# 10183308/popsift

Hardware: AMD Instinct MI355X
Metric: Mpix/s SIFT extract on 1920x1080 (keypoints+descriptors) (higher is better)
Workload: dtype f32; 1 GPU; 1920x1080 u8 grayscale, default popsift::Config (2x upscale, 9 octaves, 3 levels, PopSift mode, loop descriptor, RootSift); distinct_images_per_gpu=16, contexts_per_gpu=3, images_per_launch=16

## Files before the change

### popsift_amd/csrc/keypoint.hip

```cpp
#include <hip/hip_runtime.h>

#include "kernels.h"
#include "sift_types.h"

namespace popsift_hip {
namespace {

constexpr float F_PI = 3.14159265358979323846f;
constexpr float F_PI2 = 2.0f * 3.14159265358979323846f;
constexpr float            ORI_WINFACTOR = 1.5f;
constexpr float            DESC_MAGNIFY = 3.0f;

typedef unsigned long long fix64;
__device__ __forceinline__ fix64 to_fix(float w) { return (fix64)(unsigned int)(w * 1048576.0f); }
__device__ __forceinline__ float from_fix(fix64 v) { return (float)((double)v * (1.0 / 1048576.0)); }


__device__ __forceinline__ void wave_lds_sync()
{
    __builtin_amdgcn_fence(__ATOMIC_SEQ_CST, "wavefront");
    __builtin_amdgcn_wave_barrier();
}

__device__ __forceinline__ int wave_incl_scan(int v)
// ... 162 lines not shown
    return copysignf(2.0f - b, y);
}

__device__ __forceinline__ float atan2_bins(float y, float x)
{
    const float ax = fabsf(x), ay = fabsf(y);
    const float mx = fmaxf(fmaxf(ax, ay), 1e-30f), mn = fminf(ax, ay);
    const float r = mn * __builtin_amdgcn_rcpf(mx);
    const float s = r * r;
    float       p = fmaf(-0.01492126751691103f, s, 0.06703268736600876f);
    p = fmaf(p, s, -0.14823880791664124f);
    p = fmaf(p, s, 0.24642325937747955f);
    p = fmaf(p, s, -0.42350852489471436f);
    p = fmaf(p, s, 1.2732105255126953f);
    return octants(p * r, x, y, ax, ay);
}

__device__ __forceinline__ float atan2_bins9(float y, float x)
{
    const float ax = fabsf(x), ay = fabsf(y);
    const float mx = fmaxf(fmaxf(ax, ay), 1e-30f), mn = fminf(ax, ay);
    const float r = mn * __builtin_amdgcn_rcpf(mx);
    const float s = r * r;
    float       p = fmaf(0.026540832594037056f, s, -0.1084246039390564f);
    p = fmaf(p, s, 0.22938621044158936f);
    p = fmaf(p, s, -0.4205572307109833f);
    p = fmaf(p, s, 1.2730693817138672f);
    return octants(p * r, x, y, ax, ay);
}

typedef float v2f __attribute__((ext_vector_type(2)));
typedef __attribute__((address_space(3))) fix64 lds_fix64;
typedef __attribute__((address_space(3))) unsigned int lds_u32;

#ifndef KP_NW
#define KP_NW 1
#endif
constexpr int ORI_COPIES = 4;

__global__ __launch_bounds__(64 * KP_NW) void k_orientation(const PyrDesc* __restrict__ pdp, BatchDesc bd, SiftConsts sc,
                                                     int filtered, int hist_cap)
{
    const float* __restrict__   arena = bd.s[blockIdx.y].arena;
    Counters* __restrict__      ct = bd.s[blockIdx.y].ct;
    const InitExt* __restrict__ iext = filtered ? bd.s[blockIdx.y].iext2 : bd.s[blockIdx.y].iext;
    float* __restrict__         ohist = bd.s[blockIdx.y].ohist;
    const int n_oct = pdp->n_oct, L = pdp->L;
    constexpr int    NB = PS_ORI_NBINS + 2;
    __shared__ fix64 s_hist[KP_NW][ORI_COPIES][NB];
    const int        wave = threadIdx.x >> 6, lane = threadIdx.x & 63;
    fix64*           hall = &s_hist[wave][0][0];
    fix64*           hist = s_hist[wave][lane & (ORI_COPIES - 1)];

    __shared__ int ps[PS_MAX_OCT + 1];
    if (threadIdx.x == 0) ext_prefix(ct, sc, n_oct, ps);
    __syncthreads();
    const int total = min(ps[n_oct], hist_cap);

    for (XcdSlice sl = xcd_slice<KP_NW>(); sl.more(total); sl.s += sl.step) {
        const int g = sl.index();
        if (g >= total) continue;
        int o = 0;
        while (o + 1 < n_oct && g >= ps[o + 1]) o++;
        o = uniform(o);
        const InitExt  ie = iext[(size_t)o * sc.max_extrema + (g - uniform(ps[o]))];
        const OctDesc* od = &pdp->o[o];
// ... 170 lines not shown
        } else {
            angle_out[k] = 0.0f;
        }
    }
    return angles;
}

__device__ __forceinline__ DescRec make_desc_rec(const PyrDesc* __restrict__ pdp, const Ext& e, float angle, float cos_t, float sin_t)
{
    DescRec        r;
    const OctDesc* od = &pdp->o[e.octave];
    const int      lvl = min(max(e.lpos, 0), pdp->L - 1);
    const long long off = od->data_off + lvl * od->plane_stride;
    const float    x = e.xpos, y = e.ypos;
    const float    SBP = fabsf(DESC_MAGNIFY * e.sigma);
    const float    cell_px = (2.83f * SBP + 1.0f) * (2.83f * SBP + 1.0f);
    const int      fbits = min(max(31 - (int)ceilf(log2f(361.0f * cell_px)), 2), 14);
    const float    csbp = cos_t * SBP, ssbp = sin_t * SBP;
    const float    bsz = fabsf(csbp) + fabsf(ssbp);
    const float    ext_r = 2.5f * bsz;
    const int      xmin = max(1, (int)floorf(x - ext_r));
    const int      ymin = max(1, (int)floorf(y - ext_r));
    const int      xmax = min(od->w - 2, (int)floorf(x + ext_r) + 1);
    const int      ymax = min(od->h - 2, (int)floorf(y + ext_r) + 1);
    r.x = x;
    r.y = y;
    r.crsbp = cos_t / SBP;
    r.srsbp = sin_t / SBP;
    r.ang_bins = angle * (4.0f / F_PI);
    r.inv_c = (fabsf(r.crsbp) > 1e-20f) ? __builtin_amdgcn_rcpf(r.crsbp) : 0.0f;
    r.inv_s = (fabsf(r.srsbp) > 1e-20f) ? __builtin_amdgcn_rcpf(r.srsbp) : 0.0f;
    r.xymin = ((unsigned int)xmin & 0xffffu) | ((unsigned int)ymin << 16);
    r.xymax = ((unsigned int)xmax & 0xffffu) | ((unsigned int)ymax << 16);
    r.off_lo = (unsigned int)((unsigned long long)off & 0xffffffffull);
    r.off_hi = (unsigned int)((unsigned long long)off >> 32);
    r.misc = (unsigned int)od->pitch | ((unsigned int)fbits << 16) | ((SBP != 0.0f) ? (1u << 24) : 0u);
    return r;
}


constexpr int SCAN_ITEMS = 1;
constexpr int SCAN_CHUNK = 256 * SCAN_ITEMS;
constexpr int SCAN_LT = 256;
constexpr int SCAN_LCHUNK = SCAN_LT / 4;
constexpr int SCAN_SUB = SCAN_CHUNK / SCAN_LCHUNK;

__device__ __forceinline__ int clamped_total(const Counters* ct, const SiftConsts& sc, int n_oct)
{
    int acc = 0;
    for (int o = 0; o < n_oct; o++) acc += min(ct->ext_ct[o], sc.max_extrema);
    return acc;
}

__global__ __launch_bounds__(SCAN_LT) void k_scan_local(const PyrDesc* __restrict__ pdp, SiftConsts sc, BatchDesc bd,
                                                     int filtered, int hist_cap)
{
    const Counters* __restrict__ ct = bd.s[blockIdx.y].ct;
    const InitExt* __restrict__  iext = filtered ? bd.s[blockIdx.y].iext2 : bd.s[blockIdx.y].iext;
    const float* __restrict__    ohist = bd.s[blockIdx.y].ohist;
    Ext* __restrict__            ext = bd.s[blockIdx.y].ext;
    int* __restrict__            partial = bd.s[blockIdx.y].partial;
    static_assert(SCAN_CHUNK % SCAN_LCHUNK == 0 && SCAN_LT % 64 == 0, "four lanes per extremum, whole waves");
    __shared__ int s_wsum[SCAN_LT / 64];
    __shared__ int s_ps[PS_MAX_OCT + 1];
    const int      n_oct = pdp->n_oct;
    if (threadIdx.x == 0) ext_prefix(ct, sc, n_oct, s_ps);
    __syncthreads();
    const int total = s_ps[n_oct];
    const int tid = threadIdx.x, lane = tid & 63, wave = tid >> 6;
// ... 105 lines not shown
                    map[idx + q] = g;
                    float sn, cs;
                    sincos_cr(e.orientation[q], sn, cs);
                    rot[idx + q] = make_float2(cs, sn);
                    if (drec) drec[idx + q] = make_desc_rec(pdp, e, e.orientation[q], cs, sn);
                }
            }
            feats[g] = f;
            for (int o = 0; o < n_oct; o++)
                if (g == s_ps[o] && s_ps[o + 1] > s_ps[o]) ct->ori_ps[o] = idx;
        }
    }
    if (tid == 0 && chunk == nb - 1) {
        int last = chunk_offset;
        for (int k = 0; k < SCAN_SUB && (chunk * SCAN_SUB + k) * SCAN_LCHUNK < total; k++) last += partial[chunk * SCAN_SUB + k];
        ct->ori_total = last;
        ct->ext_total = total;
        for (int o = 0; o < PS_MAX_OCT; o++) {
            ct->ext_ct[o] = (o < n_oct) ? min(ct->ext_ct[o], sc.max_extrema) : 0;
            ct->ext_ps[o] = s_ps[o];
        }
    }
    __syncthreads();
    }
}


#ifndef DESC_NCOPY
#define DESC_NCOPY 4
#endif
constexpr int DESC_COPIES = DESC_NCOPY;
constexpr int DESC_RS = 36;
constexpr int DESC_CS = 3 * DESC_RS + 32;
constexpr int DESC_MAXROWS = 128;

__global__ __launch_bounds__(64 * KP_NW, 8) void k_descriptor(BatchDesc bd, SiftConsts sc, int desc_cap)
{
    const float* __restrict__   arena = bd.s[blockIdx.y].arena;
    const Counters* __restrict__ ct = bd.s[blockIdx.y].ct;
    const DescRec* __restrict__ drec = bd.s[blockIdx.y].drec;
    float* __restrict__         desc = bd.s[blockIdx.y].desc;
    constexpr int ROW_WORDS = (DESC_MAXROWS + 1 + 3) & ~3;
    static_assert(ROW_WORDS * 4 >= 352, "cell (-1, -1) of copy 0 stays inside the wave's LDS");
    __shared__ __attribute__((aligned(16))) unsigned int s_lds[KP_NW][ROW_WORDS + 2 * DESC_COPIES * DESC_CS];
    const int     lane = threadIdx.x & 63, wave = threadIdx.x >> 6;
    const int     cpy = lane & (DESC_COPIES - 1);
    unsigned int* rinfo = s_lds[wave];
    fix64*        hall = (fix64*)(s_lds[wave] + ROW_WORDS);
    const unsigned int rbase32 = (unsigned int)(size_t)(lds_u32*)rinfo;
    const float        hbasef = (float)(unsigned int)(size_t)(lds_fix64*)(hall + cpy * DESC_CS);
    const float        cpy8f = (float)(cpy << 3);
    const int     total = min(ct->ori_total, desc_cap);
    const int     maxrows = min(max(sc.desc_rows, 4), DESC_MAXROWS);

    for (XcdSlice sl = xcd_slice<KP_NW>(); sl.more(total); sl.s += sl.step) {
        const int d = sl.index();
        if (d >= total) continue;
        typedef unsigned int u4 __attribute__((ext_vector_type(4)));
        const u4*          rp = reinterpret_cast<const u4*>(drec + d);
        const u4           q0 = rp[0], q1 = rp[1], q2 = rp[2];
        const float        x = uniformf(__uint_as_float(q0.x)), y = uniformf(__uint_as_float(q0.y));
        const float        crsbp = uniformf(__uint_as_float(q0.z)), srsbp = uniformf(__uint_as_float(q0.w));
        const float        ang_bins = uniformf(__uint_as_float(q1.x));
        const float        inv_c = uniformf(__uint_as_float(q1.y)), inv_s = uniformf(__uint_as_float(q2.w));
        const int          pmin = uniform((int)q1.z), pmax = uniform((int)q1.w);
        const unsigned int misc = (unsigned int)uniform((int)q2.z);
        const int          pitch = (int)(misc & 0xffffu), fbits = (int)((misc >> 16) & 0xffu);
        const float*       layer = arena + uniform64((long long)(((unsigned long long)q2.y << 32) | q2.x));

        {
            u4 zero;
            asm volatile("v_mov_b32 %0, 0\n\tv_mov_b32 %1, 0\n\tv_mov_b32 %2, 0\n\tv_mov_b32 %3, 0"
                         : "=v"(zero.x), "=v"(zero.y), "=v"(zero.z), "=v"(zero.w));
            constexpr int CLEAR16 = DESC_COPIES * DESC_CS / 2;
            static_assert(DESC_COPIES * DESC_CS % 2 == 0, "whole 16-byte pieces");
            u4*           h16 = reinterpret_cast<u4*>(hall);
#pragma unroll
            for (int k = 0; k < (CLEAR16 + 63) / 64; k++)
                if (lane + 64 * k < CLEAR16) h16[lane + 64 * k] = zero;
        }

        if (misc & (1u << 24)) {
            const int   xmin = (int)(short)(pmin & 0xffff), ymin0 = pmin >> 16;
            const int   xmax = (int)(short)(pmax & 0xffff), ymax = pmax >> 16;
            const int   wx = xmax - xmin + 1;
            const int   hy_all = ymax - ymin0 + 1;
            const float ffbits = (float)fbits;

            for (int rb = 0; rb < hy_all && wx > 0; rb += maxrows) {
            const int   ymin = ymin0 + rb;
            const int   hy = min(hy_all - rb, maxrows);

            int T = 0, grow = 0;
            {
                int         carry = 0;
                for (int r0 = 0; r0 < hy; r0 += 64) {
                    const int r = r0 + lane;
                    int       len = 0, jlo = xmin;
                    if (r < hy) {
                        const float dy = (float)(ymin + r) - y;
                        const float a = srsbp * dy, b = crsbp * dy;
                        float       lo = -1e30f, hi = 1e30f;
                        bool        ok = true;
                        if (inv_c != 0.0f) {
                            const float t0 = (-2.5f - a) * inv_c, t1 = (2.5f - a) * inv_c;
                            lo = fminf(t0, t1);
                            hi = fmaxf(t0, t1);
                        } else {
                            ok = fabsf(a) < 2.5f;
                        }
                        if (inv_s != 0.0f) {
                            const float t0 = (b - 2.5f) * inv_s, t1 = (b + 2.5f) * inv_s;
                            lo = fmaxf(lo, fminf(t0, t1));
                            hi = fminf(hi, fmaxf(t0, t1));
                        } else {
                            ok = ok && (fabsf(b) < 2.5f);
                        }
                        jlo = max(xmin, (int)floorf(x + lo - 1e-3f) + 1);
                        const int jhi = min(xmax, (int)ceilf(x + hi + 1e-3f) - 1);
                        len = ok ? max(jhi - jlo + 1, 0) : 0;
                        if (len == 0) jlo = xmin;
                    }
                    const int incl = wave_incl_scan(len);
                    const int start = carry + incl - len;
                    if (r < hy) rinfo[r] = (unsigned int)start | ((unsigned int)(start - (jlo - xmin)) << 16);
                    const unsigned long long live = __ballot(len > 0);
                    if (carry == 0 && live != 0ull) grow = r0 + __ffsll((long long)live) - 1;
                    carry += __builtin_amdgcn_readlane(incl, 63);
                }
                T = carry;
                if (lane == 0) {
                    rinfo[hy] = (unsigned int)T | 0x7fff0000u;
                    rinfo[hy + 1] = 0xffffu;
                }
            }
            wave_lds_sync();

#ifdef DESC_PROBE_NOLOOP
            const int   steps = 0;
#else
            const int   steps = (T + 63) >> 6;
#endif
            unsigned int rp = rbase32 + 4u * (unsigned int)grow;
            float        fr = (float)(rb + grow);
            unsigned int cur = 0;
            unsigned int nxt = 0x7fff0000u | 0xffffu;
            if (T > 0) {
                cur = rinfo[grow];
                nxt = rinfo[grow + 1];
            }

            const float  ox = (float)xmin - x, oy = (float)ymin0 - y;
            const float  u0 = fmaf(crsbp, ox, srsbp * oy), v0 = fmaf(crsbp, oy, -srsbp * ox);
            const float* corner = layer + (size_t)(ymin0 * pitch + xmin);
            const float  pitch4f = (float)(4 * pitch);

            auto coord = [&](int i, unsigned int& off, float& u, float& v) {
                while (i >= (int)(nxt & 0xffffu)) {
                    fr += 1.0f;
                    rp += 4u;
                    cur = nxt;
                    nxt = *(lds_u32*)(size_t)(rp + 4u);
                }
                const float fc = (float)(i - ((int)cur >> 16));
                u = fmaf(crsbp, fc, fmaf(srsbp, fr, u0));
                v = fmaf(crsbp, fr, fmaf(-srsbp, fc, v0));
                asm("v_cvt_u32_f32 %0, %1" : "=v"(off) : "v"(fmaf(fr, pitch4f, fc * 4.0f)));
            };
            unsigned int probe_acc = 0u;
            auto bin = [&](float u, float v, float gx, float gy) {
                if (fabsf(u) < 2.5f && fabsf(v) < 2.5f) {
                    const float  mod = __builtin_amdgcn_sqrtf(fmaf(gx, gx, gy * gy));
                    const float  wm = __builtin_amdgcn_exp2f(fmaf(-0.18033688011112042f, fmaf(u, u, v * v), ffbits)) * mod;
                    const float tth = atan2_bins9(gy, gx) - ang_bins;
                    const float ffo = floorf(tth);
                    const float do0 = tth - ffo;

                    const float tu = u + 1.5f, tv = v + 1.5f;
                    const float fcx = floorf(tu), fcy = floorf(tv);
                    const float fx = tu - fcx, fy = tv - fcy;
                    const float wx0 = 1.0f - fx, wy0 = (1.0f - fy) * wm, wy1 = fy * wm;
                    const float w0 = 1.0f - do0;
                    const unsigned int s0 = (unsigned int)(int)fmaf(fcx, 32.0f, fmaf(ffo, 8.0f, cpy8f)) & 56u;
                    const unsigned int cb = (unsigned int)(int)fmaf(fcy, (float)(DESC_RS * 8), fmaf(fcx, 64.0f, hbasef));
                    const unsigned int e0 = cb + s0;
                    const unsigned int e1 = (s0 ^ 32u) + cb;
                    const bool x0 = tu >= 0.0f, x1 = tu < 3.0f, y0 = tv >= 0.0f, y1 = tv < 3.0f;
#ifdef DESC_PROBE_NOATOMIC
#define PS_CELL_ADD(ADDR, LO, HI) probe_acc ^= (LO) ^ (HI) ^ (ADDR);
#else
#define PS_CELL_ADD(ADDR, LO, HI)                                                                             \
    __hip_atomic_fetch_add((lds_fix64*)(size_t)(ADDR), ((fix64)(HI) << 32) | (fix64)(LO), __ATOMIC_RELAXED,    \
                           __HIP_MEMORY_SCOPE_WORKGROUP);
#endif
#define PS_CELL(ADDR, WGT)                                                                                     \
    {                                                                                                          \
        const float        wgt = (WGT);                                                                        \
        const unsigned int lo = __float_as_uint(fmaf(w0, wgt, 8388608.0f)) & 0x7fffffu;                        \
        const unsigned int hi = __float_as_uint(fmaf(do0, wgt, 8388608.0f)) & 0x7fffffu;                       \
        PS_CELL_ADD(ADDR, lo, hi)                                                                              \
    }
                    if (y0) {
                        if (x0) PS_CELL(e0, wy0 * wx0)
                        if (x1) PS_CELL(e1 + 64u, wy0 * fx)
                    }
                    if (y1) {
                        if (x0) PS_CELL(e0 + DESC_RS * 8u, wy1 * wx0)
                        if (x1) PS_CELL(e1 + DESC_RS * 8u + 64u, wy1 * fx)
                    }
#undef PS_CELL
#undef PS_CELL_ADD
                }
            };
            unsigned int off_a = 0, off_b = 0;
            float u_a = 3.0f, v_a = 3.0f, a0 = 0.0f, a1 = 0.0f, a2 = 0.0f, a3 = 0.0f;
            float u_b = 3.0f, v_b = 3.0f, b0 = 0.0f, b1 = 0.0f, b2 = 0.0f, b3 = 0.0f;
            const Taps taps(corner, pitch);
#ifdef DESC_PROBE_NOLOAD
#define PS_TAPS(OFF, A0, A1, A2, A3) { A0 = __uint_as_float(OFF) * 1e-9f; A1 = u0; A2 = v0; A3 = __uint_as_float((OFF) ^ 0x3f800000u); }
#else
#define PS_TAPS(OFF, A0, A1, A2, A3) taps.load_b(OFF, A0, A1, A2, A3);
#endif
            if (T > 0) {
                coord(lane, off_a, u_a, v_a);
                PS_TAPS(off_a, a0, a1, a2, a3)
            }
            int t = steps, i = lane;
            for (; t > 2; t -= 2, i += 128) {
                coord(i + 64, off_b, u_b, v_b);
                PS_TAPS(off_b, b0, b1, b2, b3)
                bin(u_a, v_a, a0 - a1, a2 - a3);
                coord(i + 128, off_a, u_a, v_a);
                PS_TAPS(off_a, a0, a1, a2, a3)
                bin(u_b, v_b, b0 - b1, b2 - b3);
            }
            if (t == 2) {
                coord(i + 64, off_b, u_b, v_b);
                PS_TAPS(off_b, b0, b1, b2, b3)
            }
            if (t > 0) bin(u_a, v_a, a0 - a1, a2 - a3);
            if (t == 2) bin(u_b, v_b, b0 - b1, b2 - b3);
            if (probe_acc == 0x12345u) desc[(size_t)d * 128 + lane] = 1.0f;
            wave_lds_sync();
            }
        }
        wave_lds_sync();

        fix64 a0 = 0ull, a1 = 0ull;
        {
            const int b = lane & 7, ix = (lane >> 3) & 3, iyl = lane >> 5;
#pragma unroll
            for (int k = 0; k < DESC_COPIES; k++) {
                const int sl = (b + k + ((ix & 1) << 2)) & 7, sh = (b + 7 + k + ((ix & 1) << 2)) & 7;
                const int c0 = k * DESC_CS + iyl * DESC_RS + ix * 8;
                const int c1 = k * DESC_CS + (iyl + 2) * DESC_RS + ix * 8;
                a0 += (hall[c0 + sl] & 0xffffffffull) + (hall[c0 + sh] >> 32);
                a1 += (hall[c1 + sl] & 0xffffffffull) + (hall[c1 + sh] >> 32);
            }
        }
        const float inv_scale = scalbnf(1.0f, -fbits);
        float       v0 = (float)a0 * inv_scale, v1 = (float)a1 * inv_scale;

        if (sc.norm_mode == POPSIFT_HIP_NORM_ROOTSIFT) {
            float sum = v0 + v1;
            sum = wave_allsum(sum);
            const float rs = __builtin_amdgcn_rcpf(sum);
            v0 = scalbnf(__builtin_amdgcn_sqrtf(v0 * rs), sc.norm_multi);
            v1 = scalbnf(__builtin_amdgcn_sqrtf(v1 * rs), sc.norm_multi);
        } else {
            float sq = v0 * v0 + v1 * v1;
            sq = wave_allsum(sq);
            const float norm = __builtin_amdgcn_sqrtf(sq);
            v0 = fminf(v0, 0.2f * norm);
            v1 = fminf(v1, 0.2f * norm);
            sq = v0 * v0 + v1 * v1;
            sq = wave_allsum(sq);
// ... 345 lines not shown
```

### popsift_amd/csrc/sift_types.h

```cpp
#pragma once
#include <stdint.h>

#include <hip/hip_vector_types.h>

#include "../../include/popsift_hip.h"

#define PS_MAX_OCT POPSIFT_HIP_MAX_OCTAVES
#define PS_MAX_PLANES (POPSIFT_HIP_MAX_LEVELS + 3)
#define PS_GA POPSIFT_HIP_GAUSS_ALIGN
#define PS_ORI_NBINS 36

struct OctDesc {
    float*  data;
    float*  dog;
    int64_t data_off;
    int64_t dog_off;
    int64_t plane_stride;
    int     w, h, pitch;
    int     tile_begin;
};

struct PyrDesc {
    int     n_oct;
    int     levels;
    int     L;
    int     total_tiles;
    int     dog_fly;
    int     pad_;
    OctDesc o[PS_MAX_OCT];
};

struct SiftConsts {
    float sigma0, sigma_k, edge_limit, threshold;
    int   max_extrema, norm_multi, norm_mode, sift_mode;
    int   grid_size;
    int   up_fac_int;
    int   desc_mode;
    int   det_qcap;
    int   filter_max;
    int   filter_mode;
    int   desc_rows;
};

struct InitExt {
    float xpos, ypos;
    int   lpos;
    float sigma;
    int   cell;
};

struct Ext {
    float xpos, ypos;
    int   lpos;
    float sigma;
    int   octave;
    int   num_ori;
    int   idx_ori;
    float orientation[POPSIFT_HIP_ORI_MAX];
};

struct DescRec {
    float        x, y;
    float        crsbp, srsbp;
    float        ang_bins;
    float        inv_c;
    unsigned int xymin, xymax;
    unsigned int off_lo, off_hi;
    unsigned int misc;
    float        inv_s;
};

static_assert(sizeof(DescRec) == 48, "three 16-byte loads");

struct Counters {
    int ext_ct[PS_MAX_OCT];
    int ori_ct[PS_MAX_OCT];
    int ext_ps[PS_MAX_OCT];
    int ori_ps[PS_MAX_OCT];
    int ext_total;
    int ori_total;
    int pad[2];
    struct {
        int n;
        int pad[31];
    } qcnt[64];
};
#define DET_SUBQ 64

#define PS_MAX_BATCH POPSIFT_HIP_MAX_BATCH
struct FilterState;
struct Slot {
    float*               arena;
    Counters*            ct;
    const void*          input;
    int2*                cand;
    int*                 ovf;
    InitExt*             iext;
    InitExt*             iext2;
    FilterState*         fstate;
    int*                 fhist;
    float*               ohist;
    Ext*                 ext;
    int*                 partial;
    int*                 map;
    float2*              rot;
// ... 51 lines not shown
```

### include/popsift_hip.h

```cpp
#ifndef POPSIFT_HIP_H
#define POPSIFT_HIP_H

#include <stddef.h>
#include <stdint.h>

#ifdef __cplusplus
extern "C" {
#endif

#define POPSIFT_HIP_MAX_OCTAVES 20
#define POPSIFT_HIP_MAX_LEVELS 12
#define POPSIFT_HIP_MAX_BATCH 16
#define POPSIFT_HIP_GAUSS_ALIGN 32
#define POPSIFT_HIP_ORI_MAX 4

typedef enum popsift_hip_status {
    POPSIFT_HIP_OK = 0,
    POPSIFT_HIP_ERR_INVALID = -1,
    POPSIFT_HIP_ERR_DEVICE = -2,
    POPSIFT_HIP_ERR_NO_DEVICE = -3,
    POPSIFT_HIP_ERR_OOM = -4,
    POPSIFT_HIP_ERR_STATE = -5,
    POPSIFT_HIP_ERR_TOO_SMALL = -6
} popsift_hip_status;
// ... 220 lines not shown
    uint32_t seed;
    int32_t  reserved[2];
} popsift_hip_ransac_opts;
typedef struct popsift_hip_ransac_result {
    float   H[9];
    int32_t n_inliers;
    int32_t hypothesis;
    int32_t n_valid;
    int32_t reserved;
} popsift_hip_ransac_result;
typedef struct popsift_hip_verifier popsift_hip_verifier;
int  popsift_hip_verifier_create(int device, popsift_hip_verifier** out);
int  popsift_hip_verifier_free(popsift_hip_verifier* v);
void popsift_hip_default_ransac_opts(popsift_hip_ransac_opts* o);
int  popsift_hip_ransac(popsift_hip_verifier* v, const float* pts, int n, const popsift_hip_ransac_opts* o,
                        popsift_hip_ransac_result* res, uint8_t* inlier);
int  popsift_hip_ransac_trace(popsift_hip_verifier* v, const float* pts, int n, const popsift_hip_ransac_opts* o,
                              int32_t* samples, float* models, int32_t* counts);
int  popsift_hip_pair_points(const popsift_hip_devfeatures* l, const popsift_hip_devfeatures* r,
                             const popsift_hip_pair* pairs, int n, float* pts);

int popsift_hip_get_report(const popsift_hip_ctx* ctx, popsift_hip_report* rep);
int popsift_hip_set_profile(popsift_hip_ctx* ctx, int profile);

int popsift_hip_octave_dims(const popsift_hip_ctx* ctx, int octave, int* w, int* h);
int popsift_hip_download_plane(popsift_hip_ctx* ctx, int octave, int kind, int level, float* out);
int popsift_hip_upload_plane(popsift_hip_ctx* ctx, int octave, int kind, int level, const float* in);
int popsift_hip_download_extrema(popsift_hip_ctx* ctx, popsift_hip_extremum* out, size_t cap, int* n);
int popsift_hip_rerun_keypoint_stages(popsift_hip_ctx* ctx);
enum { POPSIFT_HIP_DEBUG_DET_QCAP = 1, POPSIFT_HIP_DEBUG_CAND_CAP = 2, POPSIFT_HIP_DEBUG_OHIST_CAP = 3,
       POPSIFT_HIP_DEBUG_FAIL_ALLOC = 4, POPSIFT_HIP_DEBUG_DESC_ROWS = 5,
       POPSIFT_HIP_DEBUG_KP_WAVES = 7, POPSIFT_HIP_DEBUG_BLUR_PATH = 8, POPSIFT_HIP_DEBUG_BLUR_SEG = 9,
       POPSIFT_HIP_DEBUG_PYR_TAIL = 10, POPSIFT_HIP_DEBUG_DIRECT_PATH = 11,
       POPSIFT_HIP_DEBUG_DESC_CAP = 12, POPSIFT_HIP_DEBUG_SCALE_PATH = 13, POPSIFT_HIP_DEBUG_ORDER_COARSE = 14 };
int popsift_hip_debug_set(popsift_hip_ctx* ctx, int what, int value);

#ifdef __cplusplus
}
#endif
#endif
```

### popsift_amd/_capi.py

```python
import ctypes as C
import os

import numpy as np

_HERE = os.path.dirname(os.path.abspath(__file__))
LIB_PATH = os.environ.get("POPSIFT_HIP_LIB") or os.path.join(_HERE, "libpopsift_hip.so")

MAX_OCTAVES = 20
ORI_MAX = 4

OK = 0
ERR_INVALID, ERR_DEVICE, ERR_NO_DEVICE, ERR_OOM, ERR_STATE, ERR_TOO_SMALL = -1, -2, -3, -4, -5, -6

SIFT_POPSIFT, SIFT_OPENCV, SIFT_VLFEAT = 0, 1, 2
GAUSS_VLFEAT_COMPUTE, GAUSS_VLFEAT_RELATIVE, GAUSS_VLFEAT_RELATIVE_ALL = 0, 1, 2
GAUSS_OPENCV_COMPUTE, GAUSS_FIXED9, GAUSS_FIXED15 = 3, 4, 5
DESC_LOOP, DESC_ILOOP, DESC_GRID, DESC_IGRID, DESC_NOTILE = 0, 1, 2, 3, 4
NORM_ROOTSIFT, NORM_CLASSIC = 0, 1
SCALE_DEFAULT, SCALE_DIRECT = 0, 1
ORDER_ARRIVAL, ORDER_RASTER = 0, 1
ORDER_CHUNK = 1024


class Params(C.Structure):
# ... 111 lines not shown
    ("popsift_hip_devfeatures_download", C.c_int, [_vp, _vp, _vp]),
    ("popsift_hip_devfeatures_download_u8", C.c_int, [_vp, _vp]),
    ("popsift_hip_match_sets", C.c_int, [_vp, _vp, _vp]),
    ("popsift_hip_match_set_path", C.c_int, [C.c_int]),
    ("popsift_hip_default_match_opts", None, [C.POINTER(MatchOpts)]),
    ("popsift_hip_match_pairs", C.c_int, [_vp, _vp, C.POINTER(MatchOpts), _vp, C.c_size_t, _ip]),
    ("popsift_hip_bytefeatures_from_host", C.c_int, [C.c_int, _vp, C.c_int, C.POINTER(_vp)]),
    ("popsift_hip_bytefeatures_from_set", C.c_int, [_vp, C.POINTER(_vp)]),
    ("popsift_hip_clone_results_u8", C.c_int, [_vp, C.c_int, C.POINTER(_vp)]),
    ("popsift_hip_bytefeatures_free", C.c_int, [_vp]),
    ("popsift_hip_bytefeatures_info", C.c_int, [_vp, _ip, _ip]),
    ("popsift_hip_bytefeatures_download", C.c_int, [_vp, _vp, _vp]),
    ("popsift_hip_match_bytes", C.c_int, [_vp, _vp, _vp]),
    ("popsift_hip_match_pairs_bytes", C.c_int, [_vp, _vp, C.POINTER(MatchOpts), _vp, C.c_size_t, _ip]),
    ("popsift_hip_verifier_create", C.c_int, [C.c_int, C.POINTER(_vp)]),
    ("popsift_hip_verifier_free", C.c_int, [_vp]),
    ("popsift_hip_default_ransac_opts", None, [C.POINTER(RansacOpts)]),
    ("popsift_hip_ransac", C.c_int, [_vp, _vp, C.c_int, C.POINTER(RansacOpts), _vp, _vp]),
    ("popsift_hip_ransac_trace", C.c_int, [_vp, _vp, C.c_int, C.POINTER(RansacOpts), _vp, _vp, _vp]),
    ("popsift_hip_pair_points", C.c_int, [_vp, _vp, _vp, C.c_int, _vp]),
    ("popsift_hip_get_report", C.c_int, [_vp, C.POINTER(Report)]),
    ("popsift_hip_set_profile", C.c_int, [_vp, C.c_int]),
    ("popsift_hip_octave_dims", C.c_int, [_vp, C.c_int, _ip, _ip]),
    ("popsift_hip_download_plane", C.c_int, [_vp, C.c_int, C.c_int, C.c_int, _vp]),
    ("popsift_hip_upload_plane", C.c_int, [_vp, C.c_int, C.c_int, C.c_int, _vp]),
    ("popsift_hip_download_extrema", C.c_int, [_vp, _vp, C.c_size_t, _ip]),
    ("popsift_hip_rerun_keypoint_stages", C.c_int, [_vp]),
    ("popsift_hip_debug_set", C.c_int, [_vp, C.c_int, C.c_int]),
]
MATCH_AUTO, MATCH_EXACT, MATCH_SCREEN = 0, 1, 2
STAGES = ("pyramid", "detect", "refine", "orientation", "scan", "descriptor")
DEBUG_DET_QCAP, DEBUG_CAND_CAP, DEBUG_OHIST_CAP, DEBUG_FAIL_ALLOC, DEBUG_DESC_ROWS, DEBUG_KP_WAVES = 1, 2, 3, 4, 5, 7
DEBUG_BLUR_PATH, DEBUG_BLUR_SEG, DEBUG_PYR_TAIL, DEBUG_DIRECT_PATH, DEBUG_DESC_CAP = 8, 9, 10, 11, 12
DEBUG_SCALE_PATH, DEBUG_ORDER_COARSE = 13, 14
MAX_BATCH = 16
IMG_HOST_U8, IMG_HOST_F32, IMG_DEV_U8, IMG_DEV_F32, IMG_PINNED_U8, IMG_PINNED_F32 = range(6)

_lib = None


def _desc_type(fmt):
    if fmt == "f32":
        return np.float32
    if fmt == "u8":
        return np.uint8
    raise ValueError("fmt: 'f32' or 'u8', got %r" % (fmt,))


def quantize_u8(desc):
    d = np.asarray(desc, np.float32)
    with np.errstate(invalid="ignore"):
        pos = d > 0
        t = np.trunc(d)
        r = np.where(np.abs(d - t) >= np.float32(0.5), t + np.float32(1.0), t)
        r = np.where(d >= np.float32(255.0), np.float32(255.0), r)
        r = np.where(pos, r, np.float32(0.0))
    return r.astype(np.uint8)


class PopsiftHipError(RuntimeError):
    def __init__(self, status, where, detail=""):
        self.status = status
        msg = "%s failed: %d (%s)" % (where, status, lib().popsift_hip_strerror(status).decode())
        if detail:
            msg += ": " + detail
        super().__init__(msg)

# ... 523 lines not shown
```

### popsift_amd/csrc/ctx.hip

```cpp
#include <hip/hip_runtime.h>

#include <algorithm>
#include <atomic>
#include <cmath>
#include <cstdarg>
#include <cstddef>
#include <cstdio>
#include <cstdlib>
#include <cstring>
#include <new>
#include <type_traits>
#include <vector>

#include "devfeatures.h"
#include "kernels.h"
#include "sift_types.h"
#include "trace.h"

using namespace popsift_hip;

namespace {

constexpr int PITCH_ALIGN = 64;
constexpr int PROFILE_REPS = 4;
// ... 74 lines not shown
};

struct popsift_hip_ctx {
    int                device = 0;
    popsift_hip_params p{};
    int                levels = 3, L = 6;
    GaussRows<POPSIFT_HIP_MAX_LEVELS> tab{};
    GaussRows<POPSIFT_HIP_MAX_LEVELS> abs0{};
    float*             d_abs0 = nullptr;
    int                direct_path = 0;
    GaussRows<POPSIFT_HIP_MAX_OCTAVES> dd{};
    float*             d_dd = nullptr;
    int                scale_path = 0;
    SiftConsts         sc{};
    hipStream_t        stream = nullptr;
    hipEvent_t         ev_begin = nullptr, ev_end = nullptr;
    hipEvent_t         ev_stage[POPSIFT_HIP_STAGE_COUNT + 1] = {};

    int  in_w = 0, in_h = 0;
    int  frozen_octaves = -1;
    bool have_image = false, finished = false;
    bool batch_ok = false;
    int  nb = 1;
    bool describe = false;
    int  ori_given = 0;
    int  frames_max = 0;

    ImageSlot slot[PS_MAX_BATCH];
    BatchDesc bd{};
    PyrDesc   pd{};
    int       kp_waves = 65536;
    int       det_qcap = 1 << 30;
    int       desc_rows = 1 << 30;
    BlurTune  blur_tune{0, 0};
    int       order_coarse = 0;
    int       pyr_tail = 0;
    int       cand_cap_init = 1 << 20;
    bool      cand_cap_user = false;
    int       ohist_cap_init = 0;
    int       desc_cap_init = 0;
    size_t    ext_cap = 0;
    int       cand_cap = 0, desc_cap = 0;
    size_t    ohist_cap = 0;
    hipStream_t copy_stream = nullptr;
    hipEvent_t  ev_u8 = nullptr;
    bool     copy_pending = false;
    unsigned long submit_seq = 0, copy_seq = 0;
    Counters* d_ct = nullptr;
    Counters* h_ct = nullptr;
    PyrDesc*  d_pd = nullptr;
    PyrDesc*  h_pd = nullptr;
    int       n_feat[PS_MAX_BATCH] = {}, n_desc[PS_MAX_BATCH] = {};

    int                    fail_alloc_in = 0;
    int                    profile = 0;
    std::vector<EventPair> blur_events;
    size_t                 blur_events_used = 0;
    popsift_hip_report     rep{};

    char err[256] = {0};
};

namespace {

int fail(popsift_hip_ctx* c, int code, const char* fmt, ...)
{
// ... 79 lines not shown
    auto& a0 = c->abs0;
    memset(&a0, 0, sizeof(a0));
    if (p.gauss_mode == POPSIFT_HIP_GAUSS_VLFEAT_RELATIVE_ALL) {
        for (int lvl = 0; lvl < c->L; lvl++) {
            const float sigmaS = sigma0 * powf(2.0f, (float)lvl / (float)levels);
            a0.sigma[lvl] = sqrtf(fabsf(sigmaS * sigmaS - initial_blur * initial_blur));
        }
        compute_filter_rows(a0, p.gauss_mode);
    }
    auto& dd = c->dd;
    memset(&dd, 0, sizeof(dd));
    for (int oct = 0; oct < POPSIFT_HIP_MAX_OCTAVES; oct++) {
        const float oct_sigma = ldexpf(sigma0, oct);
        const float b = sqrtf(fabsf(oct_sigma * oct_sigma - initial_blur * initial_blur));
        dd.sigma[oct] = ldexpf(b, -oct);
    }
    compute_filter_rows(dd, p.gauss_mode);
    SiftConsts& sc = c->sc;
    sc.sigma0 = sigma0;
    sc.sigma_k = powf(2.0f, 1.0f / levels);
    sc.edge_limit = p.edge_limit;
    sc.threshold = p.threshold * 0.5f * 255.0f / levels;
    sc.max_extrema = p.max_extrema;
    sc.norm_multi = p.norm_multi;
    sc.norm_mode = p.norm_mode;
    sc.sift_mode = p.sift_mode;
    sc.grid_size = p.filter_grid_size > 0 ? p.filter_grid_size : 1;
    sc.up_fac_int = (int)p.upscale_factor;
    sc.desc_mode = p.desc_mode;
    sc.filter_max = p.filter_max_extrema;
    sc.filter_mode = p.filter_sorting;
    sc.det_qcap = c->det_qcap;
    sc.desc_rows = c->desc_rows;
}

void plan_dims(const popsift_hip_ctx* c, int w, int h, int octaves_cfg, int* n_oct, int* bw, int* bh)
{
    const float scaleFactor = 1.0f / powf(2.0f, -c->p.upscale_factor);
    int         oct = octaves_cfg;
    if (oct < 0) oct = std::max(int(floorf(logf((float)std::min(w, h)) / logf(2.0f)) - 3.0f + scaleFactor), 1);
    oct = std::min(oct, PS_MAX_OCT);
    *n_oct = oct;
    *bw = (int)ceilf(w * scaleFactor);
    *bh = (int)ceilf(h * scaleFactor);
}

hipError_t ctx_malloc(popsift_hip_ctx* c, void** p, size_t bytes)
{
    if (c->fail_alloc_in > 0 && --c->fail_alloc_in == 0) {
        *p = nullptr;
        return hipErrorOutOfMemory;
    }
    return hipMalloc(p, bytes);
}

template <class T, size_t PER>
int grow(popsift_hip_ctx* c, DevBuf<T, PER>& b, size_t need)
{
    if (need <= b.cap) return 0;
    HIP_TRY(c, b.release());
    HIP_TRY(c, ctx_malloc(c, (void**)&b.p, need * PER * sizeof(T)));
    b.cap = need;
    return 0;
}

void refresh_caps(popsift_hip_ctx* c)
// ... 1877 lines not shown
    switch (what) {
    case POPSIFT_HIP_DEBUG_DET_QCAP:
        c->det_qcap = c->sc.det_qcap = std::max(value, 0);
        return POPSIFT_HIP_OK;
    case POPSIFT_HIP_DEBUG_CAND_CAP:
        c->cand_cap_init = std::max(value, DET_SUBQ);
        c->cand_cap_user = true;
        return POPSIFT_HIP_OK;
    case POPSIFT_HIP_DEBUG_OHIST_CAP:
        c->ohist_cap_init = std::max(value, 1);
        return POPSIFT_HIP_OK;
    case POPSIFT_HIP_DEBUG_DESC_CAP:
        c->desc_cap_init = std::max(value, 0);
        return POPSIFT_HIP_OK;
    case POPSIFT_HIP_DEBUG_FAIL_ALLOC:
        c->fail_alloc_in = std::max(value, 0);
        return POPSIFT_HIP_OK;
    case POPSIFT_HIP_DEBUG_KP_WAVES:
        c->kp_waves = std::min(std::max(value / 32 * 32, 32), 1 << 20);
        return POPSIFT_HIP_OK;
    case POPSIFT_HIP_DEBUG_BLUR_PATH:
        if (value < 0 || value > 2) return fail(c, POPSIFT_HIP_ERR_INVALID, "BLUR_PATH: 0, 1 or 2");
        c->blur_tune.path = value;
        return POPSIFT_HIP_OK;
    case POPSIFT_HIP_DEBUG_BLUR_SEG:
        c->blur_tune.seg_rows = std::max(value, 0);
        return POPSIFT_HIP_OK;
    case POPSIFT_HIP_DEBUG_PYR_TAIL:
        c->pyr_tail = value;
        return POPSIFT_HIP_OK;
    case POPSIFT_HIP_DEBUG_DESC_ROWS:
        c->desc_rows = c->sc.desc_rows = std::max(value, 4);
        return POPSIFT_HIP_OK;
    case POPSIFT_HIP_DEBUG_DIRECT_PATH:
        if (value < 0 || value > 1) return fail(c, POPSIFT_HIP_ERR_INVALID, "DIRECT_PATH: 0 or 1");
        c->direct_path = value;
        return POPSIFT_HIP_OK;
    case POPSIFT_HIP_DEBUG_SCALE_PATH:
        if (value < 0 || value > 1) return fail(c, POPSIFT_HIP_ERR_INVALID, "SCALE_PATH: 0 or 1");
        c->scale_path = value;
        return POPSIFT_HIP_OK;
    case POPSIFT_HIP_DEBUG_ORDER_COARSE:
        if (value < 0 || value > 15) return fail(c, POPSIFT_HIP_ERR_INVALID, "ORDER_COARSE: 0 .. 15");
        c->order_coarse = value;
        return POPSIFT_HIP_OK;
    }
    return fail(c, POPSIFT_HIP_ERR_INVALID, "unknown debug switch %d", what);
}

int popsift_hip_rerun_keypoint_stages(popsift_hip_ctx* c)
{
    if (!c) return POPSIFT_HIP_ERR_INVALID;
    if (!c->have_image || !c->batch_ok) return fail(c, POPSIFT_HIP_ERR_STATE, "no image submitted");
    HIP_TRY(c, hipSetDevice(c->device));
    HIP_TRY(c, hipStreamSynchronize(c->stream));
    if (int rc = drain_copy(c)) return rc;
    c->blur_events_used = 0;
    HIP_TRY(c, hipEventRecord(c->ev_begin, c->stream));
    if (int rc = c->describe ? enqueue_describe_stages(c) : enqueue_keypoint_stages(c)) return rc;
    HIP_TRY(c, hipEventRecord(c->ev_end, c->stream));
    c->finished = false;
    for (ImageSlot& sl : c->slot) sl.moved = false;
    return POPSIFT_HIP_OK;
}

}
// ... 1 lines not shown
```

Measured before the change: 3735 Mpix/s.

## Precompute descriptor-origin constants per keypoint and pack row records as 64-bit

New measurement: 3728 Mpix/s. No clear change (-0.2%).

```diff
diff --git a/popsift_amd/csrc/keypoint.hip b/popsift_amd/csrc/keypoint.hip
--- a/popsift_amd/csrc/keypoint.hip
+++ b/popsift_amd/csrc/keypoint.hip
@@ -454,9 +454,15 @@
     r.inv_s = (fabsf(r.srsbp) > 1e-20f) ? __builtin_amdgcn_rcpf(r.srsbp) : 0.0f;
     r.xymin = ((unsigned int)xmin & 0xffffu) | ((unsigned int)ymin << 16);
     r.xymax = ((unsigned int)xmax & 0xffffu) | ((unsigned int)ymax << 16);
-    r.off_lo = (unsigned int)((unsigned long long)off & 0xffffffffull);
-    r.off_hi = (unsigned int)((unsigned long long)off >> 32);
+    const long long coff = off + (long long)(size_t)(ymin * od->pitch + xmin);
+    r.off_lo = (unsigned int)((unsigned long long)coff & 0xffffffffull);
+    r.off_hi = (unsigned int)((unsigned long long)coff >> 32);
     r.misc = (unsigned int)od->pitch | ((unsigned int)fbits << 16) | ((SBP != 0.0f) ? (1u << 24) : 0u);
+    const float ox = (float)xmin - x, oy = (float)ymin - y;
+    r.u0 = fmaf(r.crsbp, ox, r.srsbp * oy);
+    r.v0 = fmaf(r.crsbp, oy, -r.srsbp * ox);
+    r.pitch4f = (float)(4 * od->pitch);
+    r.ffbits = (float)fbits;
     return r;
 }
 
@@ -628,7 +634,7 @@
 constexpr int DESC_COPIES = DESC_NCOPY;
 constexpr int DESC_RS = 36;
 constexpr int DESC_CS = 3 * DESC_RS + 32;
-constexpr int DESC_MAXROWS = 128;
+constexpr int DESC_MAXROWS = 79;
 
 __global__ __launch_bounds__(64 * KP_NW, 8) void k_descriptor(BatchDesc bd, SiftConsts sc, int desc_cap)
 {
@@ -636,14 +642,15 @@
     const Counters* __restrict__ ct = bd.s[blockIdx.y].ct;
     const DescRec* __restrict__ drec = bd.s[blockIdx.y].drec;
     float* __restrict__         desc = bd.s[blockIdx.y].desc;
-    constexpr int ROW_WORDS = (DESC_MAXROWS + 1 + 3) & ~3;
+    constexpr int ROW_WORDS = (2 * (DESC_MAXROWS + 1) + 3) & ~3;
     static_assert(ROW_WORDS * 4 >= 352, "cell (-1, -1) of copy 0 stays inside the wave's LDS");
+    static_assert(DESC_COPIES > 4 || (ROW_WORDS + 2 * DESC_COPIES * DESC_CS) * 4 <= 5120, "8 waves per SIMD: 32 waves in 160 KiB");
     __shared__ __attribute__((aligned(16))) unsigned int s_lds[KP_NW][ROW_WORDS + 2 * DESC_COPIES * DESC_CS];
     const int     lane = threadIdx.x & 63, wave = threadIdx.x >> 6;
     const int     cpy = lane & (DESC_COPIES - 1);
-    unsigned int* rinfo = s_lds[wave];
+    fix64*        rrec = (fix64*)s_lds[wave];
     fix64*        hall = (fix64*)(s_lds[wave] + ROW_WORDS);
-    const unsigned int rbase32 = (unsigned int)(size_t)(lds_u32*)rinfo;
+    const unsigned int rbase32 = (unsigned int)(size_t)(lds_fix64*)rrec;
     const float        hbasef = (float)(unsigned int)(size_t)(lds_fix64*)(hall + cpy * DESC_CS);
     const float        cpy8f = (float)(cpy << 3);
     const int     total = min(ct->ori_total, desc_cap);
@@ -654,7 +661,7 @@
         if (d >= total) continue;
         typedef unsigned int u4 __attribute__((ext_vector_type(4)));
         const u4*          rp = reinterpret_cast<const u4*>(drec + d);
-        const u4           q0 = rp[0], q1 = rp[1], q2 = rp[2];
+        const u4           q0 = rp[0], q1 = rp[1], q2 = rp[2], q3 = rp[3];
         const float        x = uniformf(__uint_as_float(q0.x)), y = uniformf(__uint_as_float(q0.y));
         const float        crsbp = uniformf(__uint_as_float(q0.z)), srsbp = uniformf(__uint_as_float(q0.w));
         const float        ang_bins = uniformf(__uint_as_float(q1.x));
@@ -662,7 +669,9 @@
         const int          pmin = uniform((int)q1.z), pmax = uniform((int)q1.w);
         const unsigned int misc = (unsigned int)uniform((int)q2.z);
         const int          pitch = (int)(misc & 0xffffu), fbits = (int)((misc >> 16) & 0xffu);
-        const float*       layer = arena + uniform64((long long)(((unsigned long long)q2.y << 32) | q2.x));
+        const float*       corner = arena + uniform64((long long)(((unsigned long long)q2.y << 32) | q2.x));
+        const float        cu0 = uniformf(__uint_as_float(q3.x)), cv0 = uniformf(__uint_as_float(q3.y));
+        const float        pitch4f = uniformf(__uint_as_float(q3.z)), ffbits = uniformf(__uint_as_float(q3.w));
 
         {
             u4 zero;
@@ -681,7 +690,6 @@
             const int   xmax = (int)(short)(pmax & 0xffff), ymax = pmax >> 16;
             const int   wx = xmax - xmin + 1;
             const int   hy_all = ymax - ymin0 + 1;
-            const float ffbits = (float)fbits;
 
             for (int rb = 0; rb < hy_all && wx > 0; rb += maxrows) {
             const int   ymin = ymin0 + rb;
@@ -718,17 +726,16 @@
                         if (len == 0) jlo = xmin;
                     }
                     const int incl = wave_incl_scan(len);
-                    const int start = carry + incl - len;
-                    if (r < hy) rinfo[r] = (unsigned int)start | ((unsigned int)(start - (jlo - xmin)) << 16);
+                    const int next = carry + incl, start = next - len;
+                    if (r < hy)
+                        rrec[r] = (fix64)((unsigned int)next | ((unsigned int)(start - (jlo - xmin)) << 16)) |
+                                  ((fix64)__float_as_uint((float)(rb + r)) << 32);
                     const unsigned long long live = __ballot(len > 0);
                     if (carry == 0 && live != 0ull) grow = r0 + __ffsll((long long)live) - 1;
                     carry += __builtin_amdgcn_readlane(incl, 63);
                 }
                 T = carry;
-                if (lane == 0) {
-                    rinfo[hy] = (unsigned int)T | 0x7fff0000u;
-                    rinfo[hy + 1] = 0xffffu;
-                }
+                if (lane == 0) rrec[hy] = (fix64)(0xffffu | 0x7fff0000u);
             }
             wave_lds_sync();
 
@@ -737,30 +744,27 @@
 #else
             const int   steps = (T + 63) >> 6;
 #endif
-            unsigned int rp = rbase32 + 4u * (unsigned int)grow;
-            float        fr = (float)(rb + grow);
-            unsigned int cur = 0;
-            unsigned int nxt = 0x7fff0000u | 0xffffu;
+            unsigned int rp = rbase32 + 8u * (unsigned int)grow;
+            unsigned int cw = 0xffffu | 0x7fff0000u, cf = 0u;
             if (T > 0) {
-                cur = rinfo[grow];
-                nxt = rinfo[grow + 1];
+                const fix64 rec = rrec[grow];
+                cw = (unsigned int)rec;
+                cf = (unsigned int)(rec >> 32);
             }
 
-            const float  ox = (float)xmin - x, oy = (float)ymin0 - y;
-            const float  u0 = fmaf(crsbp, ox, srsbp * oy), v0 = fmaf(crsbp, oy, -srsbp * ox);
-            const float* corner = layer + (size_t)(ymin0 * pitch + xmin);
-            const float  pitch4f = (float)(4 * pitch);
 
             auto coord = [&](int i, unsigned int& off, float& u, float& v) {
-                while (i >= (int)(nxt & 0xffffu)) {
-                    fr += 1.0f;
-                    rp += 4u;
-                    cur = nxt;
-                    nxt = *(lds_u32*)(size_t)(rp + 4u);
+                while (i >= (int)(cw & 0xffffu)) {
+                    rp += 8u;
+                    const fix64 rec = *(lds_fix64*)(size_t)rp;
+                    cw = (unsigned int)rec;
+                    cf = (unsigned int)(rec >> 32);
                 }
-                const float fc = (float)(i - ((int)cur >> 16));
-                u = fmaf(crsbp, fc, fmaf(srsbp, fr, u0));
-                v = fmaf(crsbp, fr, fmaf(-srsbp, fc, v0));
+                asm volatile("" : "+v"(cw), "+v"(cf));
+                const float fr = __uint_as_float(cf);
+                const float fc = (float)(i - ((int)cw >> 16));
+                u = fmaf(crsbp, fc, fmaf(srsbp, fr, cu0));
+                v = fmaf(crsbp, fr, fmaf(-srsbp, fc, cv0));
                 asm("v_cvt_u32_f32 %0, %1" : "=v"(off) : "v"(fmaf(fr, pitch4f, fc * 4.0f)));
             };
             unsigned int probe_acc = 0u;
@@ -813,7 +817,7 @@
             float u_b = 3.0f, v_b = 3.0f, b0 = 0.0f, b1 = 0.0f, b2 = 0.0f, b3 = 0.0f;
             const Taps taps(corner, pitch);
 #ifdef DESC_PROBE_NOLOAD
-#define PS_TAPS(OFF, A0, A1, A2, A3) { A0 = __uint_as_float(OFF) * 1e-9f; A1 = u0; A2 = v0; A3 = __uint_as_float((OFF) ^ 0x3f800000u); }
+#define PS_TAPS(OFF, A0, A1, A2, A3) { A0 = __uint_as_float(OFF) * 1e-9f; A1 = cu0; A2 = cv0; A3 = __uint_as_float((OFF) ^ 0x3f800000u); }
 #else
 #define PS_TAPS(OFF, A0, A1, A2, A3) taps.load_b(OFF, A0, A1, A2, A3);
 #endif
diff --git a/popsift_amd/csrc/sift_types.h b/popsift_amd/csrc/sift_types.h
--- a/popsift_amd/csrc/sift_types.h
+++ b/popsift_amd/csrc/sift_types.h
@@ -68,9 +68,12 @@
     unsigned int off_lo, off_hi;
     unsigned int misc;
     float        inv_s;
+    float        u0, v0;
+    float        pitch4f;
+    float        ffbits;
 };
 
-static_assert(sizeof(DescRec) == 48, "three 16-byte loads");
+static_assert(sizeof(DescRec) == 64, "four 16-byte loads");
 
 struct Counters {
     int ext_ct[PS_MAX_OCT];
```

## Replace per-row while-loop lookup in descriptor with bitmask popcount row indexing

Applied to the files above, without the earlier changes.

Measured after the change: 3644 Mpix/s before, 3785 Mpix/s after (median of 6 runs). +3.9%, better.

```diff
diff --git a/include/popsift_hip.h b/include/popsift_hip.h
--- a/include/popsift_hip.h
+++ b/include/popsift_hip.h
@@ -276,7 +276,8 @@
        POPSIFT_HIP_DEBUG_FAIL_ALLOC = 4, POPSIFT_HIP_DEBUG_DESC_ROWS = 5,
        POPSIFT_HIP_DEBUG_KP_WAVES = 7, POPSIFT_HIP_DEBUG_BLUR_PATH = 8, POPSIFT_HIP_DEBUG_BLUR_SEG = 9,
        POPSIFT_HIP_DEBUG_PYR_TAIL = 10, POPSIFT_HIP_DEBUG_DIRECT_PATH = 11,
-       POPSIFT_HIP_DEBUG_DESC_CAP = 12, POPSIFT_HIP_DEBUG_SCALE_PATH = 13, POPSIFT_HIP_DEBUG_ORDER_COARSE = 14 };
+       POPSIFT_HIP_DEBUG_DESC_CAP = 12, POPSIFT_HIP_DEBUG_SCALE_PATH = 13, POPSIFT_HIP_DEBUG_ORDER_COARSE = 14,
+       POPSIFT_HIP_DEBUG_DESC_LIST = 15 };
 int popsift_hip_debug_set(popsift_hip_ctx* ctx, int what, int value);
 
 #ifdef __cplusplus
diff --git a/popsift_amd/_capi.py b/popsift_amd/_capi.py
--- a/popsift_amd/_capi.py
+++ b/popsift_amd/_capi.py
@@ -167,7 +167,7 @@
 STAGES = ("pyramid", "detect", "refine", "orientation", "scan", "descriptor")
 DEBUG_DET_QCAP, DEBUG_CAND_CAP, DEBUG_OHIST_CAP, DEBUG_FAIL_ALLOC, DEBUG_DESC_ROWS, DEBUG_KP_WAVES = 1, 2, 3, 4, 5, 7
 DEBUG_BLUR_PATH, DEBUG_BLUR_SEG, DEBUG_PYR_TAIL, DEBUG_DIRECT_PATH, DEBUG_DESC_CAP = 8, 9, 10, 11, 12
-DEBUG_SCALE_PATH, DEBUG_ORDER_COARSE = 13, 14
+DEBUG_SCALE_PATH, DEBUG_ORDER_COARSE, DEBUG_DESC_LIST = 13, 14, 15
 MAX_BATCH = 16
 IMG_HOST_U8, IMG_HOST_F32, IMG_DEV_U8, IMG_DEV_F32, IMG_PINNED_U8, IMG_PINNED_F32 = range(6)
 
diff --git a/popsift_amd/csrc/ctx.hip b/popsift_amd/csrc/ctx.hip
--- a/popsift_amd/csrc/ctx.hip
+++ b/popsift_amd/csrc/ctx.hip
@@ -130,6 +130,7 @@
     int       kp_waves = 65536;
     int       det_qcap = 1 << 30;
     int       desc_rows = 1 << 30;
+    int       desc_list = 1 << 30;
     BlurTune  blur_tune{0, 0};
     int       order_coarse = 0;
     int       pyr_tail = 0;
@@ -275,6 +276,7 @@
     sc.filter_mode = p.filter_sorting;
     sc.det_qcap = c->det_qcap;
     sc.desc_rows = c->desc_rows;
+    sc.desc_list = c->desc_list;
 }
 
 void plan_dims(const popsift_hip_ctx* c, int w, int h, int octaves_cfg, int* n_oct, int* bw, int* bh)
@@ -2218,6 +2220,9 @@
     case POPSIFT_HIP_DEBUG_DESC_ROWS:
         c->desc_rows = c->sc.desc_rows = std::max(value, 4);
         return POPSIFT_HIP_OK;
+    case POPSIFT_HIP_DEBUG_DESC_LIST:
+        c->desc_list = c->sc.desc_list = std::max(value, 64);
+        return POPSIFT_HIP_OK;
     case POPSIFT_HIP_DEBUG_DIRECT_PATH:
         if (value < 0 || value > 1) return fail(c, POPSIFT_HIP_ERR_INVALID, "DIRECT_PATH: 0 or 1");
         c->direct_path = value;
diff --git a/popsift_amd/csrc/keypoint.hip b/popsift_amd/csrc/keypoint.hip
--- a/popsift_amd/csrc/keypoint.hip
+++ b/popsift_amd/csrc/keypoint.hip
@@ -218,6 +218,8 @@
 typedef float v2f __attribute__((ext_vector_type(2)));
 typedef __attribute__((address_space(3))) fix64 lds_fix64;
 typedef __attribute__((address_space(3))) unsigned int lds_u32;
+typedef __attribute__((address_space(3))) short lds_i16;
+typedef __attribute__((address_space(3))) unsigned long long lds_u64;
 
 #ifndef KP_NW
 #define KP_NW 1
@@ -628,7 +630,10 @@
 constexpr int DESC_COPIES = DESC_NCOPY;
 constexpr int DESC_RS = 36;
 constexpr int DESC_CS = 3 * DESC_RS + 32;
-constexpr int DESC_MAXROWS = 128;
+constexpr int DESC_MAXROWS = 96;
+constexpr int DESC_REC_WORDS = (((DESC_MAXROWS + 1) * 2 + 7) / 8) * 2;
+constexpr int DESC_TAB64 = 55;
+constexpr int DESC_LISTCAP = (DESC_TAB64 - 1) * 64;
 
 __global__ __launch_bounds__(64 * KP_NW, 8) void k_descriptor(BatchDesc bd, SiftConsts sc, int desc_cap)
 {
@@ -636,18 +641,24 @@
     const Counters* __restrict__ ct = bd.s[blockIdx.y].ct;
     const DescRec* __restrict__ drec = bd.s[blockIdx.y].drec;
     float* __restrict__         desc = bd.s[blockIdx.y].desc;
-    constexpr int ROW_WORDS = (DESC_MAXROWS + 1 + 3) & ~3;
+    constexpr int ROW_WORDS = DESC_REC_WORDS + 2 * DESC_TAB64;
+    static_assert(ROW_WORDS % 4 == 0 && DESC_REC_WORDS % 2 == 0, "the histograms start on a 16-byte boundary, the table on an 8-byte one");
     static_assert(ROW_WORDS * 4 >= 352, "cell (-1, -1) of copy 0 stays inside the wave's LDS");
+    static_assert((ROW_WORDS + 2 * DESC_COPIES * DESC_CS) * 4 <= 5120, "32 waves per CU share 160 KiB");
+    static_assert(DESC_TAB64 <= 64, "one lane clears one word of the table");
     __shared__ __attribute__((aligned(16))) unsigned int s_lds[KP_NW][ROW_WORDS + 2 * DESC_COPIES * DESC_CS];
     const int     lane = threadIdx.x & 63, wave = threadIdx.x >> 6;
     const int     cpy = lane & (DESC_COPIES - 1);
-    unsigned int* rinfo = s_lds[wave];
+    short*        rec = (short*)s_lds[wave];
+    unsigned int* tab = s_lds[wave] + DESC_REC_WORDS;
     fix64*        hall = (fix64*)(s_lds[wave] + ROW_WORDS);
-    const unsigned int rbase32 = (unsigned int)(size_t)(lds_u32*)rinfo;
+    const unsigned int rbase32 = (unsigned int)(size_t)(lds_i16*)rec;
+    const unsigned int tbase32 = (unsigned int)(size_t)(lds_u32*)tab;
     const float        hbasef = (float)(unsigned int)(size_t)(lds_fix64*)(hall + cpy * DESC_CS);
     const float        cpy8f = (float)(cpy << 3);
     const int     total = min(ct->ori_total, desc_cap);
     const int     maxrows = min(max(sc.desc_rows, 4), DESC_MAXROWS);
+    const int     maxlist = min(max(sc.desc_list, 64), DESC_LISTCAP);
 
     for (XcdSlice sl = xcd_slice<KP_NW>(); sl.more(total); sl.s += sl.step) {
         const int d = sl.index();
@@ -683,11 +694,14 @@
             const int   hy_all = ymax - ymin0 + 1;
             const float ffbits = (float)fbits;
 
-            for (int rb = 0; rb < hy_all && wx > 0; rb += maxrows) {
+            for (int rb = 0, skip = 0; rb < hy_all && wx > 0;) {
             const int   ymin = ymin0 + rb;
             const int   hy = min(hy_all - rb, maxrows);
-
-            int T = 0, grow = 0;
+            if (lane < DESC_TAB64) ((unsigned long long*)tab)[lane] = 0ull;
+            wave_lds_sync();
+
+            int T = 0, grow = 0, nrec = 0;
+            int rb_next = rb + hy, skip_next = 0;
             {
                 int         carry = 0;
                 for (int r0 = 0; r0 < hy; r0 += 64) {
@@ -715,20 +729,47 @@
                         jlo = max(xmin, (int)floorf(x + lo - 1e-3f) + 1);
                         const int jhi = min(xmax, (int)ceilf(x + hi + 1e-3f) - 1);
                         len = ok ? max(jhi - jlo + 1, 0) : 0;
+                        if (r == 0) {
+                            const int s = min(skip, len);
+                            jlo += s;
+                            len -= s;
+                        }
                         if (len == 0) jlo = xmin;
                     }
+                    const unsigned long long live = __ballot(len > 0);
+                    bool                     below = carry > 0;
+                    if (carry == 0 && live != 0ull) {
+                        const int first = __ffsll((long long)live) - 1;
+                        grow = r0 + first;
+                        below = lane > first;
+                    }
+                    if (below && r < hy && len == 0) len = 1;
                     const int incl = wave_incl_scan(len);
                     const int start = carry + incl - len;
-                    if (r < hy) rinfo[r] = (unsigned int)start | ((unsigned int)(start - (jlo - xmin)) << 16);
-                    const unsigned long long live = __ballot(len > 0);
-                    if (carry == 0 && live != 0ull) grow = r0 + __ffsll((long long)live) - 1;
+                    const unsigned long long over = __ballot(carry + incl > maxlist);
+                    if (over != 0ull) {
+                        const int cut = __ffsll((long long)over) - 1;
+                        if (lane == cut) len = maxlist - start;
+                        if (lane > cut) len = 0;
+                        rb_next = rb + r0 + cut;
+                        skip_next = __builtin_amdgcn_readlane(len, cut) + ((r0 + cut == 0) ? skip : 0);
+                    }
+                    if (len > 0) {
+                        const int last = start + len - 1;
+                        rec[r - grow] = (short)((jlo - xmin) - start);
+                        __hip_atomic_fetch_or((lds_u32*)(size_t)(tbase32 + 4u * (unsigned int)(last >> 5)), 1u << (last & 31),
+                                              __ATOMIC_RELAXED, __HIP_MEMORY_SCOPE_WORKGROUP);
+                    }
+                    const unsigned long long kept = __ballot(len > 0);
+                    if (kept != 0ull) nrec = r0 + 64 - __builtin_clzll(kept) - grow;
+                    if (over != 0ull) {
+                        carry = maxlist;
+                        break;
+                    }
                     carry += __builtin_amdgcn_readlane(incl, 63);
                 }
                 T = carry;
-                if (lane == 0) {
-                    rinfo[hy] = (unsigned int)T | 0x7fff0000u;
-                    rinfo[hy + 1] = 0xffffu;
-                }
+                if (lane == 0) rec[nrec] = -32767;
             }
             wave_lds_sync();
 
@@ -737,28 +778,25 @@
 #else
             const int   steps = (T + 63) >> 6;
 #endif
-            unsigned int rp = rbase32 + 4u * (unsigned int)grow;
-            float        fr = (float)(rb + grow);
-            unsigned int cur = 0;
-            unsigned int nxt = 0x7fff0000u | 0xffffu;
-            if (T > 0) {
-                cur = rinfo[grow];
-                nxt = rinfo[grow + 1];
-            }
+            unsigned long long rmask = *(const unsigned long long*)tab;
+            unsigned int       rnext = tbase32 + 8u;
+            unsigned int       rows_done = (unsigned int)(rb + grow);
+            const unsigned int rec0 = rbase32 - 2u * (unsigned int)(rb + grow);
 
             const float  ox = (float)xmin - x, oy = (float)ymin0 - y;
             const float  u0 = fmaf(crsbp, ox, srsbp * oy), v0 = fmaf(crsbp, oy, -srsbp * ox);
             const float* corner = layer + (size_t)(ymin0 * pitch + xmin);
             const float  pitch4f = (float)(4 * pitch);
 
-            auto coord = [&](int i, unsigned int& off, float& u, float& v) {
-                while (i >= (int)(nxt & 0xffffu)) {
-                    fr += 1.0f;
-                    rp += 4u;
-                    cur = nxt;
-                    nxt = *(lds_u32*)(size_t)(rp + 4u);
-                }
-                const float fc = (float)(i - ((int)cur >> 16));
+            auto coord = [&](int i, unsigned int ahead, unsigned int& off, float& u, float& v) {
+                const unsigned int lo = (unsigned int)rmask, hi = (unsigned int)(rmask >> 32);
+                const unsigned int row = __builtin_amdgcn_mbcnt_hi(hi, __builtin_amdgcn_mbcnt_lo(lo, rows_done));
+                asm("v_bcnt_u32_b32 %0, %1, %0" : "+v"(rows_done) : "v"(lo));
+                asm("v_bcnt_u32_b32 %0, %1, %0" : "+v"(rows_done) : "v"(hi));
+                rmask = *(lds_u64*)(size_t)(rnext + ahead);
+                const int   rcd = *(lds_i16*)(size_t)(rec0 + 2u * row);
+                const float fr = (float)row;
+                const float fc = (float)(i + rcd);
                 u = fmaf(crsbp, fc, fmaf(srsbp, fr, u0));
                 v = fmaf(crsbp, fr, fmaf(-srsbp, fc, v0));
                 asm("v_cvt_u32_f32 %0, %1" : "=v"(off) : "v"(fmaf(fr, pitch4f, fc * 4.0f)));
@@ -818,26 +856,30 @@
 #define PS_TAPS(OFF, A0, A1, A2, A3) taps.load_b(OFF, A0, A1, A2, A3);
 #endif
             if (T > 0) {
-                coord(lane, off_a, u_a, v_a);
+                coord(lane, 0u, off_a, u_a, v_a);
+                rnext += 8u;
                 PS_TAPS(off_a, a0, a1, a2, a3)
             }
             int t = steps, i = lane;
             for (; t > 2; t -= 2, i += 128) {
-                coord(i + 64, off_b, u_b, v_b);
+                coord(i + 64, 0u, off_b, u_b, v_b);
                 PS_TAPS(off_b, b0, b1, b2, b3)
                 bin(u_a, v_a, a0 - a1, a2 - a3);
-                coord(i + 128, off_a, u_a, v_a);
+                coord(i + 128, 8u, off_a, u_a, v_a);
                 PS_TAPS(off_a, a0, a1, a2, a3)
                 bin(u_b, v_b, b0 - b1, b2 - b3);
+                rnext += 16u;
             }
             if (t == 2) {
-                coord(i + 64, off_b, u_b, v_b);
+                coord(i + 64, 0u, off_b, u_b, v_b);
                 PS_TAPS(off_b, b0, b1, b2, b3)
             }
             if (t > 0) bin(u_a, v_a, a0 - a1, a2 - a3);
             if (t == 2) bin(u_b, v_b, b0 - b1, b2 - b3);
             if (probe_acc == 0x12345u) desc[(size_t)d * 128 + lane] = 1.0f;
             wave_lds_sync();
+            rb = rb_next;
+            skip = skip_next;
             }
         }
         wave_lds_sync();
diff --git a/popsift_amd/csrc/sift_types.h b/popsift_amd/csrc/sift_types.h
--- a/popsift_amd/csrc/sift_types.h
+++ b/popsift_amd/csrc/sift_types.h
@@ -40,6 +40,7 @@
     int   filter_max;
     int   filter_mode;
     int   desc_rows;
+    int   desc_list;
 };
 
 struct InitExt {
```
